# KatherLab/STAMP

Measured on AMD Instinct MI355X. Metric: tiles/sec encoded (224x224, ViT-L/14), higher is better.
Workload: dtype f16

## Files before the change

stamp_amd/csrc/api.hip:

```cpp
#include "gemm_kernel.h"
#include <stdlib.h>
#include <atomic>
#include <mutex>

namespace amds {

static thread_local char g_err[512] = "";

void set_error(const char* fmt, ...) {
    va_list ap;
    va_start(ap, fmt);
    vsnprintf(g_err, sizeof(g_err), fmt, ap);
    va_end(ap);
}

int hip_fail(hipError_t e, const char* what) {
    set_error("HIP error %d (%s) in %s", (int)e, hipGetErrorString(e), what);
    return AMDS_ERR_HIP;
}

}
struct amds_ctx {
    int device = -1;
    int refs = 0;
// ... 294 lines not shown
    set_error("amds_gemm_batched: bad dtype %d", dtype);
    return AMDS_ERR_INVALID;
}

extern "C" int amds_wgrad_tn(const void* dy, long ld_dy, const void* x, long ld_x, long tokens, int N, int K, int split_k, int dtype, float* part,
                             void* stream) {
    AMDS_REQUIRE(dy && x && part, "amds_wgrad_tn: null pointer");
    AMDS_REQUIRE(tokens > 0 && N > 0 && K > 0 && split_k > 0 && split_k <= 65535, "amds_wgrad_tn: bad shape");
    AMDS_REQUIRE(N % 256 == 0 && K % 256 == 0, "amds_wgrad_tn: needs N %% 256 == 0 and K %% 256 == 0 (N=%d K=%d)", N, K);
    AMDS_REQUIRE(ld_dy % 8 == 0 && ld_x % 8 == 0 && ld_dy >= N && ld_x >= K, "amds_wgrad_tn: bad pitches");
    AMDS_REQUIRE(((uintptr_t)dy & 15) == 0 && ((uintptr_t)x & 15) == 0 && ((uintptr_t)part & 15) == 0, "amds_wgrad_tn: pointers must be 16-byte aligned");
    const long unit = 64L * split_k;
    const long chunk = (tokens + unit - 1) / unit * 64;
    AMDS_REQUIRE((chunk + 63) * std::max(ld_dy, ld_x) * 2 < (1L << 31), "amds_wgrad_tn: one split's operand span is beyond the 2 GB a buffer descriptor addresses (raise split_k)");
    EpiArgs ep;
    ep.out = part; ep.ldo = K; ep.bias = nullptr; ep.scale = nullptr; ep.pos = nullptr; ep.np = ep.T = ep.P = 0; ep.acc_scale = 1.0f;
    ep.bsA = chunk * ld_dy; ep.bsW = chunk * ld_x; ep.bsOut = (long)N * K; ep.nbatch = split_k; ep.ktot = tokens;
    hipStream_t st = (hipStream_t)stream;
    ProfScope prof(PROF_GEMM, 2.0 * tokens * (double)N * K, st);
    if (dtype == AMDS_F16) return gemm_dispatch<f16>(15, AMDS_EPI_BIAS_F32, dy, ld_dy, x, ld_x, N, K, (int)chunk, ep, st);
    if (dtype == AMDS_BF16) return gemm_dispatch<bf16>(15, AMDS_EPI_BIAS_F32, dy, ld_dy, x, ld_x, N, K, (int)chunk, ep, st);
    set_error("amds_wgrad_tn: bad dtype %d", dtype);
    return AMDS_ERR_INVALID;
}

extern "C" int amds_gemm_lnfold(const void* A, long lda, const void* W, long ldw, int M, int N, int K, int dtype, int epi, void* out,
                                long ldo, const float* bias, const float* scale, void* xh, float* rowpart, const float* rowstat,
                                const float* colsum, void* stream) {
    AMDS_REQUIRE(A && W && out, "amds_gemm_lnfold: null pointer");
    AMDS_REQUIRE(M >= 0 && N > 0 && K > 0 && K % 64 == 0 && N % 256 == 0, "amds_gemm_lnfold: needs K %% 64 == 0 and N %% 256 == 0 (M=%d N=%d K=%d)", M, N, K);
    AMDS_REQUIRE(lda % 8 == 0 && ldw % 8 == 0 && lda >= K && ldw >= K && ldo % 4 == 0, "amds_gemm_lnfold: bad pitches");
    AMDS_REQUIRE(((uintptr_t)A & 15) == 0 && ((uintptr_t)W & 15) == 0 && ((uintptr_t)out & 15) == 0 && ((uintptr_t)xh & 15) == 0,
                 "amds_gemm_lnfold: pointers must be 16-byte aligned");
    const bool producer = xh || rowpart, consumer = rowstat || colsum;
    AMDS_REQUIRE(producer != consumer, "amds_gemm_lnfold: either (xh, rowpart) [RESIDUAL] or (rowstat, colsum) [BIAS / BIAS_GELU / SWIGLU]");
    if (producer) {
        AMDS_REQUIRE(epi == AMDS_EPI_RESIDUAL && xh && rowpart, "amds_gemm_lnfold: the producer form is the RESIDUAL epilogue with xh AND rowpart");
    } else {
        AMDS_REQUIRE((epi == AMDS_EPI_BIAS || epi == AMDS_EPI_BIAS_GELU || epi == AMDS_EPI_SWIGLU) && rowstat && colsum && bias,
                     "amds_gemm_lnfold: the consumer form is BIAS / BIAS_GELU / SWIGLU with rowstat, colsum AND bias");
    }
    if (M == 0) return AMDS_OK;
    EpiArgs ep;
    ep.out = out; ep.ldo = ldo; ep.bias = bias; ep.scale = scale; ep.pos = nullptr; ep.np = ep.T = ep.P = 0; ep.acc_scale = 1.0f;
    ep.xh = xh; ep.rowpart = rowpart; ep.rowstat = rowstat; ep.colsum = colsum;
    hipStream_t st = (hipStream_t)stream;
    ProfScope prof(PROF_GEMM, 2.0 * M * (double)N * K, st);
    if (dtype == AMDS_F16) return gemm_dispatch<f16>(12, epi, A, lda, W, ldw, M, N, K, ep, st);
    if (dtype == AMDS_BF16) return gemm_dispatch<bf16>(12, epi, A, lda, W, ldw, M, N, K, ep, st);
    set_error("amds_gemm_lnfold: bad dtype %d", dtype);
    return AMDS_ERR_INVALID;
}

extern "C" int amds_gemm_lnfold_planes(const void* A, long lda, const void* W, long ldw, int M, int N, int K, void* hi, void* lo, long ld,
                                       const float* bias, const float* scale, float* rowpart, void* stream) {
    AMDS_REQUIRE(A && W && hi && lo && rowpart, "amds_gemm_lnfold_planes: null pointer");
    AMDS_REQUIRE(M >= 0 && N > 0 && K > 0 && K % 64 == 0 && N % 256 == 0, "amds_gemm_lnfold_planes: needs K %% 64 == 0 and N %% 256 == 0 (M=%d N=%d K=%d)", M, N, K);
    AMDS_REQUIRE(lda % 8 == 0 && ldw % 8 == 0 && lda >= K && ldw >= K && ld % 4 == 0 && ld >= N, "amds_gemm_lnfold_planes: bad pitches");
    AMDS_REQUIRE(((uintptr_t)A & 15) == 0 && ((uintptr_t)W & 15) == 0 && ((uintptr_t)hi & 15) == 0 && ((uintptr_t)lo & 15) == 0,
                 "amds_gemm_lnfold_planes: pointers must be 16-byte aligned");
    AMDS_REQUIRE(hi != lo && A != hi && A != lo, "amds_gemm_lnfold_planes: the planes are updated in place and must not alias each other or A");
    if (M == 0) return AMDS_OK;
    EpiArgs ep;
    ep.out = hi; ep.ldo = ld; ep.bias = bias; ep.scale = scale; ep.pos = nullptr; ep.np = ep.T = ep.P = 0; ep.acc_scale = 1.0f;
    ep.xh = hi; ep.xl = lo; ep.rowpart = rowpart;
    hipStream_t st = (hipStream_t)stream;
    ProfScope prof(PROF_GEMM, 2.0 * M * (double)N * K, st);
    return gemm_dispatch<f16>(12, AMDS_EPI_RESIDUAL, A, lda, W, ldw, M, N, K, ep, st);
}

extern "C" long amds_gemm_persist_launches(void) { return g_gemm_persist_launches.load(std::memory_order_relaxed); }

extern "C" int amds_gemm_ex(int cfg, const void* A, long lda, const void* W, long ldw, int M, int N, int K, int dtype,
                            int epi, void* out, long ldo, const float* bias, const float* scale, const float* pos,
                            int np, int T, int P, float acc_scale, void* stream) {
    return gemm_impl(cfg, A, lda, W, ldw, M, N, K, dtype, epi, out, ldo, bias, scale, pos, np, T, P, acc_scale, stream);
}
```

stamp_amd/csrc/common.h:

```cpp
#pragma once
#include <type_traits>
#include <hip/hip_runtime.h>
#include <stdint.h>
#include <stdio.h>
#include <stdarg.h>
#include <string.h>
#include <atomic>
#include "../../include/amdstamp.h"

namespace amds {

typedef _Float16 f16;
typedef __bf16 bf16;
typedef _Float16 f16x4 __attribute__((ext_vector_type(4)));
typedef _Float16 f16x8 __attribute__((ext_vector_type(8)));
typedef __bf16 bf16x4 __attribute__((ext_vector_type(4)));
typedef __bf16 bf16x8 __attribute__((ext_vector_type(8)));
typedef float f32x4 __attribute__((ext_vector_type(4)));
typedef float f32x16 __attribute__((ext_vector_type(16)));
typedef unsigned int u32x4 __attribute__((ext_vector_type(4)));
typedef unsigned int u32x2 __attribute__((ext_vector_type(2)));
typedef int i32x4 __attribute__((ext_vector_type(4)));

void set_error(const char* fmt, ...);
// ... 124 lines not shown
}
__device__ __forceinline__ f32x2 gelu_erf_poly2(f32x2 x) {
    f32x2 q[1] = {x};
    gelu_erf_poly2_n<1>(q);
    return q[0];
}
__device__ __forceinline__ float silu(float x) { return x * __builtin_amdgcn_rcpf(1.0f + __expf(-x)); }
__device__ __forceinline__ f32x2 silu_mul2(f32x2 g, f32x2 v) {
    const f32x2 a = g * f32x2{-1.44269504088896340736f, -1.44269504088896340736f};
    const f32x2 d = f32x2{__builtin_amdgcn_exp2f(a[0]), __builtin_amdgcn_exp2f(a[1])} + f32x2{1.0f, 1.0f};
    return g * f32x2{__builtin_amdgcn_rcpf(d[0]), __builtin_amdgcn_rcpf(d[1])} * v;
}

__device__ __forceinline__ float half_wave_sum(float v) {
    v += __builtin_bit_cast(float, __builtin_amdgcn_update_dpp(0, __builtin_bit_cast(int, v), 0xB1, 0xF, 0xF, true));
    v += __builtin_bit_cast(float, __builtin_amdgcn_update_dpp(0, __builtin_bit_cast(int, v), 0x4E, 0xF, 0xF, true));
    v += __builtin_bit_cast(float, __builtin_amdgcn_update_dpp(0, __builtin_bit_cast(int, v), 0x141, 0xF, 0xF, true));
    v += __builtin_bit_cast(float, __builtin_amdgcn_update_dpp(0, __builtin_bit_cast(int, v), 0x140, 0xF, 0xF, true));
    v += __builtin_bit_cast(float, __builtin_amdgcn_ds_swizzle(__builtin_bit_cast(int, v), 0x401F));
    return v;
}
__device__ __forceinline__ f32x2 half_wave_sum8(const f32x2 (&v)[8], int lane) {
    auto dpp = [](float x, auto ctrl_c) {
        return __builtin_bit_cast(float, __builtin_amdgcn_update_dpp(0, __builtin_bit_cast(int, x), decltype(ctrl_c)::value, 0xF, 0xF, true));
    };
    typedef std::integral_constant<int, 0x140> MIRROR;
    typedef std::integral_constant<int, 0x141> HALF_MIRROR;
    typedef std::integral_constant<int, 0xB1> XOR1;
    typedef std::integral_constant<int, 0x4E> XOR2;
    const bool b3 = lane & 8, b2 = lane & 4;
    f32x2 a[4], b[2], c;
#pragma unroll
    for (int j = 0; j < 4; ++j)
#pragma unroll
        for (int e = 0; e < 2; ++e) {
            float lo = v[j][e], hi4 = v[4 + j][e];
            asm volatile("s_nop 1\n\tv_permlane16_swap_b32 %0, %1\n\ts_nop 1" : "+v"(lo), "+v"(hi4));
            a[j][e] = lo + hi4;
        }
#pragma unroll
    for (int j = 0; j < 2; ++j) {
        const f32x2 keep = b3 ? a[2 + j] : a[j], send = b3 ? a[j] : a[2 + j];
        b[j] = keep + f32x2{dpp(send[0], MIRROR{}), dpp(send[1], MIRROR{})};
    }
    {
        const f32x2 keep = b2 ? b[1] : b[0], send = b2 ? b[0] : b[1];
        c = keep + f32x2{dpp(send[0], HALF_MIRROR{}), dpp(send[1], HALF_MIRROR{})};
    }
    c += f32x2{dpp(c[0], XOR1{}), dpp(c[1], XOR1{})};
    c += f32x2{dpp(c[0], XOR2{}), dpp(c[1], XOR2{})};
    return c;
}

__device__ __forceinline__ float half_wave_max(float v) {
    v = fmaxf(v, __builtin_bit_cast(float, __builtin_amdgcn_update_dpp(0, __builtin_bit_cast(int, v), 0xB1, 0xF, 0xF, true)));
    v = fmaxf(v, __builtin_bit_cast(float, __builtin_amdgcn_update_dpp(0, __builtin_bit_cast(int, v), 0x4E, 0xF, 0xF, true)));
    v = fmaxf(v, __builtin_bit_cast(float, __builtin_amdgcn_update_dpp(0, __builtin_bit_cast(int, v), 0x141, 0xF, 0xF, true)));
    v = fmaxf(v, __builtin_bit_cast(float, __builtin_amdgcn_update_dpp(0, __builtin_bit_cast(int, v), 0x140, 0xF, 0xF, true)));
    v = fmaxf(v, __builtin_bit_cast(float, __builtin_amdgcn_ds_swizzle(__builtin_bit_cast(int, v), 0x401F)));
    return v;
}

__device__ __forceinline__ float wave_sum(float v) {
#pragma unroll
    for (int o = 32; o > 0; o >>= 1) v += __shfl_xor(v, o, 64);
    return v;
}
__device__ __forceinline__ float wave_max(float v) {
#pragma unroll
    for (int o = 32; o > 0; o >>= 1) v = fmaxf(v, __shfl_xor(v, o, 64));
    return v;
}

__device__ __forceinline__ float dist_sqrt(float x) { return __builtin_amdgcn_sqrtf(x); }
__device__ __host__ __forceinline__ uint32_t fmix32(uint32_t h) {
    h ^= h >> 16; h *= 0x85EBCA6Bu; h ^= h >> 13; h *= 0xC2B2AE35u; h ^= h >> 16;
    return h;
}
__device__ __host__ __forceinline__ uint32_t drop_rowkey(uint64_t seed, uint32_t stream, uint64_t row) {
    const uint32_t a = fmix32((uint32_t)seed ^ (uint32_t)row ^ (stream * 0x9E3779B1u));
    return fmix32(a + (uint32_t)(seed >> 32) + (uint32_t)(row >> 32) * 0x7FEB352Du);
}
__device__ __host__ __forceinline__ uint32_t drop_mix(uint32_t h) {
    h ^= h >> 16; h *= 0xC2B2AE35u; h ^= h >> 16;
    return h;
}
__device__ __host__ __forceinline__ uint32_t drop_pair_bits(uint32_t rowkey, uint32_t pair) { return drop_mix(rowkey ^ (pair * 0x9E3779B1u)); }
__device__ __host__ __forceinline__ bool drop_keep(uint32_t pair_bits, int odd, uint32_t thr16) {
    return ((pair_bits >> (odd ? 16 : 0)) & 0xFFFFu) >= thr16;
}
__device__ __forceinline__ bool drop_keep_flat(uint64_t seed, uint32_t stream, long idx, uint32_t thr16) {
    const uint32_t key = drop_rowkey(seed, stream, (uint64_t)(idx >> 16));
    return drop_keep(drop_pair_bits(key, (uint32_t)(idx & 0xFFFF) >> 1), (int)(idx & 1), thr16);
}
static inline uint32_t drop_thr16(float p) { const long t = lroundf(p * 65536.0f); return (uint32_t)(t < 0 ? 0 : (t > 65535 ? 65535 : t)); }
static inline float drop_scale(uint32_t thr16) { return 65536.0f / (float)(65536u - thr16); }

typedef const __attribute__((address_space(1))) void* gptr_t;
typedef __attribute__((address_space(3))) void* lptr_t;
__device__ __forceinline__ void glds16(const void* g, void* lds_wave_base) {
    __builtin_amdgcn_global_load_lds((gptr_t)g, (lptr_t)lds_wave_base, 16, 0, 0);
}

__device__ __forceinline__ void bufl16(__amdgpu_buffer_rsrc_t rsrc, void* lds_wave_base, int voffset, int soffset) {
    __builtin_amdgcn_raw_ptr_buffer_load_lds(rsrc, (lptr_t)lds_wave_base, 16, voffset, soffset, 0, 0);
}
// ... 56 lines not shown
```

stamp_amd/csrc/gemm_4w16.h:

```cpp
#pragma once
#include <algorithm>
#include <type_traits>
#include "gemm_kernel.h"

namespace amds {

__device__ __forceinline__ f32x4 agpr_read(const f32x4& a) {
    f32x4 v;
    asm("v_accvgpr_read_b32 %0, %1" : "=v"(v[0]) : "a"(a[0]));
    asm("v_accvgpr_read_b32 %0, %1" : "=v"(v[1]) : "a"(a[1]));
    asm("v_accvgpr_read_b32 %0, %1" : "=v"(v[2]) : "a"(a[2]));
    asm("v_accvgpr_read_b32 %0, %1" : "=v"(v[3]) : "a"(a[3]));
    return v;
}

template <int N> struct NextTilePieces : std::integral_constant<int, N> {};
template <typename C> struct is_next_tile : std::false_type {};
template <int N> struct is_next_tile<NextTilePieces<N>> : std::true_type {};

template <typename T, int EPI, int P3 = 6, int P0 = 6, bool SPREAD = true, int PRL = 0, int PRS = 0, bool STREAM = false, bool PERSIST = false, bool TN = false>
__global__ void __launch_bounds__(256) __attribute__((amdgpu_waves_per_eu(1, 1)))
gemm_4w16_kernel(const T* __restrict__ A, long lda, const T* __restrict__ W, long ldw, int M, int N, int K,
                 EpiArgs ep, int tiles_m, int tiles_n) {
    typedef typename Act<T>::vec8 vec8;
    typedef typename Act<T>::vec4 vec4;
    constexpr int BM = 256, BN = 256, BK = 64, NT = 256;
    constexpr int ROWB = BK * 2;
    constexpr int A_BYTES = BM * ROWB, STAGE = (BM + BN) * ROWB;
    constexpr int FI = 8, FJ = 8;
    constexpr int GROUP_M = 8;

    extern __shared__ __attribute__((aligned(16))) char smem[];
#ifdef AMDS_GEMM_TRACE
    unsigned long long tr_t[4] = {0, 0, 0, 0}, tr_rt0 = __builtin_amdgcn_s_memrealtime();
    int tr_round = 0;
#define AMDS_GEMM_STAMP(k)                             \
    do {                                               \
        __builtin_amdgcn_sched_barrier(0);             \
        tr_t[k] = __builtin_amdgcn_s_memtime();        \
        __builtin_amdgcn_sched_barrier(0);             \
    } while (0)
#define AMDS_GEMM_TRACE_WRITE()                                                                                                            \
    do {                                                                                                                                   \
        if (ep.pos != nullptr && threadIdx.x == 0) {                                                                                       \
            unsigned long long* rec = reinterpret_cast<unsigned long long*>(const_cast<float*>(ep.pos)) +                                  \
                                      ((long)blockIdx.x * ((ntiles + (int)gridDim.x - 1) / (int)gridDim.x) + tr_round) * 8;                \
            rec[0] = tr_t[0]; rec[1] = tr_t[1]; rec[2] = tr_t[2]; rec[3] = tr_t[3];                                                        \
            rec[4] = (unsigned long long)__builtin_amdgcn_s_getreg(63492) | ((unsigned long long)__builtin_amdgcn_s_getreg(63508) << 32);  \
            rec[5] = (unsigned long long)ti;                                                                                               \
            rec[6] = tr_rt0; rec[7] = __builtin_amdgcn_s_memrealtime();                                                                    \
        }                                                                                                                                  \
        ++tr_round;                                                                                                                        \
    } while (0)
    AMDS_GEMM_STAMP(0);
#else
#define AMDS_GEMM_STAMP(k) do { } while (0)
#define AMDS_GEMM_TRACE_WRITE() do { } while (0)
#endif

    const int tid = threadIdx.x;
    const int lane = tid & 63;
    const int wave = __builtin_amdgcn_readfirstlane(tid >> 6);
    const int wm = wave >> 1, wn = wave & 1;
    const int l15 = lane & 15, kb = lane >> 4;
    const int l31 = lane & 31, hi = lane >> 5;

    static_assert(!PERSIST || (STREAM && !TN && P3 >= 0 && PRL + PRS == 0 && (EPI == AMDS_EPI_BIAS || EPI == AMDS_EPI_BIAS_GELU || EPI == AMDS_EPI_BIAS_RELU)),
                  "gemm_4w16: the persistent form is the streamed 16-bit epilogue on SCHED 0");
    int tm, tn;
    auto tile_of = [&](int bid, int nwg, int& tm_, int& tn_) {
        const int xcd = bid & 7, q = nwg >> 3, r = nwg & 7;
        const int t = (xcd < r ? xcd * (q + 1) : r * (q + 1) + (xcd - r) * q) + (bid >> 3);
        const int group = GROUP_M * tiles_n;
        const int g = t / group, first_m = g * GROUP_M;
        const int gm = min(tiles_m - first_m, GROUP_M);
        const int rr = t - g * group;
        tm_ = first_m + rr % gm;
        tn_ = rr / gm;
    };
    const int ntiles = PERSIST ? tiles_m * tiles_n : (int)gridDim.x;
    int ti = blockIdx.x;
    tile_of(ti, ntiles, tm, tn);
    int m0 = tm * BM, n0 = tn * BN;
    int par = 0;
    if (ep.nbatch > 1) {
        const long by = blockIdx.y;
        A += by * ep.bsA;
        W += by * ep.bsW;
        constexpr bool F32O = (EPI == AMDS_EPI_RESIDUAL || EPI == AMDS_EPI_BIAS_F32 || EPI == AMDS_EPI_BIAS_GELU_F32 || EPI == AMDS_EPI_BIAS_RELU_F32);
        if (F32O) ep.out = reinterpret_cast<float*>(ep.out) + by * ep.bsOut;
        else ep.out = reinterpret_cast<T*>(ep.out) + by * ep.bsOut;
    }

    int rows_a = min(BM, M - m0);
    const long tn_valid = TN ? (ep.ktot > 0 ? min((long)K, ep.ktot - (long)blockIdx.y * K) : (long)K) : 0;
    __amdgpu_buffer_rsrc_t rsrc_a = TN ? __builtin_amdgcn_make_buffer_rsrc(const_cast<T*>(A + m0), 0, tn_valid > 0 ? (int)(((tn_valid - 1) * lda + BM) * 2) : 0, 0x00020000)
                                             : __builtin_amdgcn_make_buffer_rsrc(const_cast<T*>(A + (long)m0 * lda), 0, (int)((((long)rows_a - 1) * lda + K) * 2), 0x00020000);
    __amdgpu_buffer_rsrc_t rsrc_w = TN ? __builtin_amdgcn_make_buffer_rsrc(const_cast<T*>(W + n0), 0, tn_valid > 0 ? (int)(((tn_valid - 1) * ldw + BN) * 2) : 0, 0x00020000)
                                             : __builtin_amdgcn_make_buffer_rsrc(const_cast<T*>(W + (long)n0 * ldw), 0, (int)(((long)(BN - 1) * ldw + K) * 2), 0x00020000);
    int voff[16];
#pragma unroll
    for (int it = 0; it < 16; ++it) {
        if constexpr (TN) {
            const int c = (it & 7) * NT + tid, row = c >> 5, pos = c & 31, g = (row & 3) | ((row >> 1) & 4);
            voff[it] = (int)(((long)row * (it < 8 ? lda : ldw) + (pos ^ (g << 1)) * 8) * 2);
        } else {
            const int c = (it & 7) * NT + tid, row = c >> 3, cp = c & 7, sc = cp ^ ((row >> 1) & 7);
            voff[it] = (int)(((long)row * (it < 8 ? lda : ldw) + sc * 8) * 2);
        }
    }
    auto issue_to = [&](const __amdgpu_buffer_rsrc_t& ra, const __amdgpu_buffer_rsrc_t& rw, char* st, int koff, int koff_w, int lo, int hi_) {
#pragma unroll
        for (int it = 0; it < 16; ++it)
            if (it >= lo && it < hi_) {
                if (it < 8) {
                    __builtin_amdgcn_raw_ptr_buffer_load_lds(ra, (lptr_t)(st + ((it & 7) * NT + wave * 64) * 16), 16, voff[it], koff, 0, 0);
                } else {
                    __builtin_amdgcn_raw_ptr_buffer_load_lds(rw, (lptr_t)(st + A_BYTES + ((it & 7) * NT + wave * 64) * 16), 16, voff[it], koff_w,
                                                             0, 0);
                }
            }
// ... 292 lines not shown
    for (int i = 0; i < FI; ++i) {
        if (i == 0)
            asm volatile("s_nop 15\n\ts_nop 15" : "+a"(acc[i][0]), "+a"(acc[i][1]), "+a"(acc[i][2]), "+a"(acc[i][3]), "+a"(acc[i][4]),
                         "+a"(acc[i][5]), "+a"(acc[i][6]), "+a"(acc[i][7]));
        else
            asm volatile("" : "+a"(acc[i][0]), "+a"(acc[i][1]), "+a"(acc[i][2]), "+a"(acc[i][3]), "+a"(acc[i][4]), "+a"(acc[i][5]),
                         "+a"(acc[i][6]), "+a"(acc[i][7]));
    }
    __builtin_amdgcn_sched_barrier(0);

    constexpr bool F16OUT = (EPI == AMDS_EPI_BIAS || EPI == AMDS_EPI_BIAS_GELU || EPI == AMDS_EPI_BIAS_RELU);
    static_assert(epi_is_staged<EPI>() || EPI == AMDS_EPI_SWIGLU, "gemm_4w16: staged epilogues and SWIGLU");
    if constexpr (EPI == AMDS_EPI_SWIGLU) {
        const float as = ep.acc_scale;
#pragma unroll
        for (int i = 0; i < FI; ++i) {
            const int row = wm * 128 + i * 16 + l15;
#pragma unroll
            for (int q = 0; q < 2; ++q)
#pragma unroll
                for (int t = 0; t < 2; ++t) {
                    f32x4 gt = agpr_read(acc[i][4 * q + t]), vl = agpr_read(acc[i][4 * q + 2 + t]);
                    if (lnf) {
                        gt = gt * rs[i][0] + (cs[4 * q + t] * rs[i][1] + cb[4 * q + t]);
                        vl = vl * rs[i][0] + (cs[4 * q + 2 + t] * rs[i][1] + cb[4 * q + 2 + t]);
                    } else if (!bias_in_acc) {
                        const f32x4 bg = *reinterpret_cast<const f32x4*>(ep.bias + n0 + wn * 128 + (4 * q + t) * 16 + 4 * kb);
                        const f32x4 bv = *reinterpret_cast<const f32x4*>(ep.bias + n0 + wn * 128 + (4 * q + 2 + t) * 16 + 4 * kb);
                        gt = gt * as + bg;
                        vl = vl * as + bv;
                    }
                    f32x4 o;
                    {
                        const f32x2 o01 = silu_mul2(f32x2{gt[0], gt[1]}, f32x2{vl[0], vl[1]}), o23 = silu_mul2(f32x2{gt[2], gt[3]}, f32x2{vl[2], vl[3]});
                        o = f32x4{o01[0], o01[1], o23[0], o23[1]};
                    }
                    const int hcol = wn * 64 + q * 32 + t * 16 + 4 * kb;
                    const int chunk = hcol >> 3, half = ((hcol >> 2) & 1) * 8;
                    *reinterpret_cast<vec4*>(smem + row * 256 + ((chunk ^ (row & 15)) << 4) + half) = Act<T>::from_f32x4(o);
                }
        }
        __syncthreads();
        const int l15r = lane & 15, rsub = lane >> 4;
#pragma unroll 4
        for (int it = 0; it < 16; ++it) {
            const int row = wave * 64 + it * 4 + rsub;
            const u32x4 v = *reinterpret_cast<const u32x4*>(smem + row * 256 + l15r * 16);
            const int chunk = l15r ^ (row & 15);
            if (m0 + row < M)
                *reinterpret_cast<u32x4*>(reinterpret_cast<T*>(ep.out) + (long)(m0 + row) * ep.ldo + n0 / 2 + chunk * 8) = v;
        }
        return;
    }
    if constexpr (EPI == AMDS_EPI_RESIDUAL) {
        if (rmw_fast) {
            const int rows_o = min(BM, M - m0);
            rsrc_o = __builtin_amdgcn_make_buffer_rsrc(reinterpret_cast<float*>(ep.out) + (long)m0 * ep.ldo + n0, 0,
                                                       (int)((((long)rows_o - 1) * ep.ldo + BN) * 4), 0x00020000);
#pragma unroll
            for (int h = 0; h < 2; ++h)
#pragma unroll
                for (int u = 0; u < 8; ++u)
                    offu[h][u] = (wave * 64 + 2 * u + hi) * ldo4 + (((l31 >> 4) ^ h) << 9) + (((l31 & 15) ^ (2 * u + hi)) << 4);
            const __amdgpu_buffer_rsrc_t rsrc_h = __builtin_amdgcn_make_buffer_rsrc(
                ep.xh ? reinterpret_cast<T*>(ep.xh) + (long)m0 * ep.ldo + n0 : reinterpret_cast<T*>(ep.out), 0,
                ep.xh ? (int)((((long)rows_o - 1) * ep.ldo + BN) * 2) : 0, 0x00020000);
            const __amdgpu_buffer_rsrc_t rsrc_l = __builtin_amdgcn_make_buffer_rsrc(
                ep.xl ? reinterpret_cast<T*>(ep.xl) + (long)m0 * ep.ldo + n0 : reinterpret_cast<T*>(ep.out), 0,
                ep.xl ? (int)((((long)rows_o - 1) * ep.ldo + BN) * 2) : 0, 0x00020000);
            const int np_part = N / 128;
            auto run = [&](auto has_scale_c, auto lnp_c, auto pl_c) {
                constexpr bool HS = decltype(has_scale_c)::value, LNP = decltype(lnp_c)::value, PL = decltype(pl_c)::value;
                auto load_prev = [&](int pass, int b8) {
                    if constexpr (PL) {
                        int rowoff = b8 * 16 * ldo4 + pass * 256;
                        asm volatile("" : "+s"(rowoff));
#pragma unroll
                        for (int u = 0; u < 8; ++u) {
                            const int o = (offu[b8 & 1][u] + rowoff) >> 1;
                            const u32x2 ph = __builtin_bit_cast(u32x2, __builtin_amdgcn_raw_buffer_load_b64(rsrc_h, o, 0, 0));
                            const u32x2 pl = __builtin_bit_cast(u32x2, __builtin_amdgcn_raw_buffer_load_b64(rsrc_l, o, 0, 0));
                            old[b8][u] = __builtin_bit_cast(f32x4, u32x4{ph[0], ph[1], pl[0], pl[1]});
                        }
                    } else {
                        load_old(pass, b8);
                    }
                };
                f32x4 sc[4];
                auto load_scale = [&](int pass) {
                    if constexpr (HS) {
#pragma unroll
                        for (int jj = 0; jj < 4; ++jj)
                            sc[jj] = *reinterpret_cast<const f32x4*>(ep.scale + n0 + wn * 128 + (pass * 4 + jj) * 16 + 4 * kb);
                    }
                };
                load_scale(0);
#pragma unroll
                for (int b8 = 0; b8 < 4; ++b8) load_prev(0, b8);
#pragma unroll
                for (int pass = 0; pass < 2; ++pass) {
#pragma unroll
                    for (int i = 0; i < FI; ++i) {
                        const int row = wm * 128 + i * 16 + l15;
#pragma unroll
                        for (int jj = 0; jj < 4; ++jj) {
                            f32x4 v = agpr_read(acc[i][pass * 4 + jj]);
// ... 29 lines not shown
                                } else {
                                    old4 = __builtin_convertvector(h4, f32x4) + __builtin_convertvector(l4, f32x4);
                                }
                                v[u] += old4;
                            } else {
                                v[u] += old[b8][u];
                                __builtin_amdgcn_raw_buffer_store_b128(__builtin_bit_cast(u32x4, v[u]), rsrc_o, offu[b8 & 1][u] + rowoff, 0, 0);
                            }
                        }
                        if constexpr (LNP) {
                            f32x2 ss[8];
#pragma unroll
                            for (int u = 0; u < 8; ++u) {
                                const vec4 c = Act<T>::from_f32x4(v[u]);
                                __builtin_amdgcn_raw_buffer_store_b64(__builtin_bit_cast(u32x2, c), rsrc_h, (offu[b8 & 1][u] + rowoff) >> 1, 0, 0);
                                if constexpr (PL) {
                                    f32x4 rest;
                                    if constexpr (std::is_same<T, f16>::value) {
                                        const u32x2 cu = __builtin_bit_cast(u32x2, c);
                                        rest = f32x4{mix_sub_fh<0>(v[u][0], cu[0]), mix_sub_fh<1>(v[u][1], cu[0]), mix_sub_fh<0>(v[u][2], cu[1]), mix_sub_fh<1>(v[u][3], cu[1])};
                                    } else {
                                        rest = v[u] - __builtin_convertvector(c, f32x4);
                                    }
                                    const vec4 cl = Act<T>::from_f32x4(rest);
                                    __builtin_amdgcn_raw_buffer_store_b64(__builtin_bit_cast(u32x2, cl), rsrc_l, (offu[b8 & 1][u] + rowoff) >> 1, 0, 0);
                                }
                                ss[u] = f32x2{(v[u][0] + v[u][1]) + (v[u][2] + v[u][3]),
                                              fmaf(v[u][0], v[u][0], v[u][1] * v[u][1]) + fmaf(v[u][2], v[u][2], v[u][3] * v[u][3])};
                            }
                            const f32x2 tot = half_wave_sum8(ss, l31);
                            const int urow = ((l31 >> 4) & 1) * 4 + ((l31 >> 3) & 1) * 2 + ((l31 >> 2) & 1);
                            const int prow = m0 + wave * 64 + b8 * 16 + 2 * urow + hi;
                            if ((l31 & 3) == 0 && prow < M)
                                *reinterpret_cast<f32x2*>(ep.rowpart + ((long)prow * np_part + tn * 2 + pass) * 2) = tot;
                        }
                        if (pass == 0) load_prev(1, b8);
                        __builtin_amdgcn_sched_barrier(0);
                    }
                    if (pass == 0) {
                        asm volatile("s_waitcnt lgkmcnt(0)" ::: "memory");
                        __builtin_amdgcn_sched_barrier(0);
                        __builtin_amdgcn_s_barrier();
                        __builtin_amdgcn_sched_barrier(0);
                    }
                }
            };
            if (ep.xl) {
                if (ep.scale) run(std::true_type{}, std::true_type{}, std::true_type{}); else run(std::false_type{}, std::true_type{}, std::true_type{});
            } else if (ep.xh) {
                if (ep.scale) run(std::true_type{}, std::true_type{}, std::false_type{}); else run(std::false_type{}, std::true_type{}, std::false_type{});
            } else {
                if (ep.scale) run(std::true_type{}, std::false_type{}, std::false_type{}); else run(std::false_type{}, std::false_type{}, std::false_type{});
            }
            return;
        }
    }
    if constexpr (F16OUT && STREAM) {
        EpiArgs epv = ep;
        if (bias_in_acc || lnf) epv.bias = nullptr;
        EpiCols<FJ> cols;
        if constexpr (PERSIST) {
#pragma unroll
            for (int j = 0; j < FJ; ++j) asm volatile("" : "=v"(cols.bias[j]));
        }
        epi_cols_load<EPI>(epv, cols, [&](int j) { return n0 + wn * 128 + j * 16 + 4 * kb; });
        if constexpr (PERSIST) {
            __builtin_amdgcn_sched_barrier(0);
            __builtin_amdgcn_s_waitcnt(0x0F70);
            __builtin_amdgcn_sched_barrier(0);
        }
        const int rows_o = min(BM, M - m0);
        const __amdgpu_buffer_rsrc_t rsrc_s = __builtin_amdgcn_make_buffer_rsrc(reinterpret_cast<T*>(ep.out) + (long)m0 * ep.ldo + n0, 0,
                                                                                (int)((((long)rows_o - 1) * ep.ldo + BN) * 2), 0x00020000);
        char* slab = smem + (PERSIST ? ((nk - 1 + par) & 1) * STAGE : 0) + wave * 8192;
        int wr_base = l15 * 256 + (((kb & 1) ^ (l15 & 1)) << 3);
        int wr_x = (kb >> 1) ^ ((l15 >> 1) & 7);
        int rd_base = kb * 512 + ((l15 ^ kb) << 4);
        int ldo2 = (int)ep.ldo * 2;
        int st_base = (wm * 128 + 2 * kb) * ldo2 + (wn * 128 + l15 * 8) * 2;
        if constexpr (PERSIST) {
            asm volatile("" : "+v"(wr_base), "+v"(wr_x), "+v"(rd_base), "+v"(st_base), "+s"(ldo2));
        }
        auto run = [&](auto mode_c) {
            constexpr int MODE = decltype(mode_c)::value;
            u32x4 rd[4];
            f32x4 b0n[PERSIST && MODE == 1 ? FJ : 1];
            if constexpr (PERSIST && MODE == 1) {
#pragma unroll
                for (int j = 0; j < FJ; ++j) b0n[j] = f32x4{0.f, 0.f, 0.f, 0.f};
                if (bias_in_acc) {
#pragma unroll
                    for (int j = 0; j < FJ; ++j) b0n[j] = *reinterpret_cast<const f32x4*>(ep.bias + n0n + wn * 128 + j * 16 + 4 * kb);
                }
            }
#pragma unroll
            for (int s = 0; s <= FI; ++s) {
                if (s < FI) {
                    char* wp = slab + (s & 1) * 4096 + wr_base;
#pragma unroll
                    for (int j = 0; j < FJ; j += 2) {
                        f32x4 v0 = agpr_read(acc[s][j]), v1 = agpr_read(acc[s][j + 1]);
                        if constexpr (MODE == 2) {
                            if constexpr (LNC) {
                                v0 = v0 * rs[s][0] + (cs[j] * rs[s][1] + cb[j]);
                                v1 = v1 * rs[s][0] + (cs[j + 1] * rs[s][1] + cb[j + 1]);
                                epi_value_pair<EPI, true, true>(epv, cb[j], cb[j], cb[j + 1], cb[j + 1], v0, v1);
// ... 131 lines not shown
                u32x4 v[8];
#pragma unroll
                for (int u = 0; u < 8; ++u) {
                    const int row = wave * 64 + (b8 * 8 + u) * 2 + hi;
                    v[u] = *reinterpret_cast<const u32x4*>(smem + row * 512 + l31 * 16);
                    if ((u >> 2) & 1) v[u] = u32x4{v[u][2], v[u][3], v[u][0], v[u][1]};
                }
#pragma unroll
                for (int u = 0; u < 8; ++u) {
                    const int row = wave * 64 + (b8 * 8 + u) * 2 + hi;
                    const int chunk = l31 ^ (row & 31);
                    if (m0 + row < M)
                        *reinterpret_cast<u32x4*>(reinterpret_cast<T*>(ep.out) + (long)(m0 + row) * ep.ldo + n0 + chunk * 8) = v[u];
                }
            } else {
                f32x4 v[8], o[8];
#pragma unroll
                for (int u = 0; u < 8; ++u) {
                    const int row = wave * 64 + (b8 * 8 + u) * 2 + hi;
                    const int chunk = l31 ^ (row & 31);
                    const int n = n0 + (chunk >> 4) * 128 + pass * 64 + (chunk & 15) * 4;
                    v[u] = *reinterpret_cast<const f32x4*>(smem + row * 512 + l31 * 16);
                    if constexpr (EPI == AMDS_EPI_RESIDUAL)
                        o[u] = *reinterpret_cast<const f32x4*>(reinterpret_cast<const float*>(ep.out) +
                                                               (long)min(m0 + row, M - 1) * ep.ldo + n);
                }
#pragma unroll
                for (int u = 0; u < 8; ++u) {
                    const int row = wave * 64 + (b8 * 8 + u) * 2 + hi;
                    const int chunk = l31 ^ (row & 31);
                    const int n = n0 + (chunk >> 4) * 128 + pass * 64 + (chunk & 15) * 4;
                    if constexpr (EPI == AMDS_EPI_RESIDUAL) v[u] += o[u];
                    if (m0 + row < M)
                        *reinterpret_cast<f32x4*>(reinterpret_cast<float*>(ep.out) + (long)(m0 + row) * ep.ldo + n) = v[u];
                }
            }
        }
    }
}

static inline int gemm_persist_grid(int tiles) {
    int g = device_cu_count() & ~7;
    const char* e = getenv("AMDS_GEMM_PERSIST_WGS");
    if (e && *e) g = std::min(g, atoi(e) & ~7);
    return std::min(tiles, std::max(g, 8));
}

template <typename T, int EPI, bool SPREAD = true, int P3 = 6, int P0 = 6, int PRL = 0, int PRS = 0, bool STREAM = false, bool PERSIST = false, bool TN = false>
static int launch_gemm_4w16(const void* A, long lda, const void* W, long ldw, int M, int N, int K, const EpiArgs& ep,
                            hipStream_t st) {
    if constexpr (!epi_is_staged<EPI>() && EPI != AMDS_EPI_SWIGLU) {
        return launch_gemm_4w64<T, EPI>(A, lda, W, ldw, M, N, K, ep, st);
    } else {
        constexpr int LDS = 2 * (256 + 256) * 128;
        constexpr bool STR = STREAM && (EPI == AMDS_EPI_BIAS || EPI == AMDS_EPI_BIAS_GELU || EPI == AMDS_EPI_BIAS_RELU);
        if constexpr (STR) {
            if (ep.ldo * 512 >= (1L << 31)) return launch_gemm_4w16<T, EPI, SPREAD, P3, P0, PRL, PRS, false, false, TN>(A, lda, W, ldw, M, N, K, ep, st);
        }
        constexpr bool PER = PERSIST && STR && !TN && P3 >= 0 && PRL + PRS == 0;
        if constexpr (PER) {
            if (ep.nbatch != 1) return launch_gemm_4w16<T, EPI, SPREAD, P3, P0, PRL, PRS, STREAM, false, TN>(A, lda, W, ldw, M, N, K, ep, st);
        }
        constexpr auto kern = gemm_4w16_kernel<T, EPI, P3, P0, SPREAD, PRL, PRS, STR, PER, TN>;
        EpiArgs epp = ep;
        if constexpr (PRL + PRS > 0) {
            static char* scratch = nullptr;
            static size_t scratch_bytes = 0;
            const size_t need = (size_t)cdiv(M, 256) * (N / 256) * (K / 64) * 4096 * (PRL > PRS ? PRL : PRS);
            if (need > scratch_bytes) {
                if (scratch) AMDS_HIP(hipFree(scratch));
                AMDS_HIP(hipMalloc(reinterpret_cast<void**>(&scratch), need));
                scratch_bytes = need;
            }
            epp.pos = reinterpret_cast<const float*>(scratch);
        }
        AMDS_HIP(lds_opt_in<kern>(LDS));
        const int tiles_m = cdiv(M, 256), tiles_n = N / 256;
        int grid = tiles_m * tiles_n;
        if constexpr (PER) {
            grid = gemm_persist_grid(grid);
            g_gemm_persist_launches.fetch_add(1, std::memory_order_relaxed);
        }
        hipLaunchKernelGGL(kern, dim3(grid, ep.nbatch), dim3(256), LDS, st, reinterpret_cast<const T*>(A), lda,
                           reinterpret_cast<const T*>(W), ldw, M, N, K, epp, tiles_m, tiles_n);
        AMDS_LAUNCH_CHECK("gemm_4w16_kernel");
        return AMDS_OK;
    }
}

}
```

stamp_amd/csrc/gemm_kernel.h:

```cpp
#pragma once
#include <stdlib.h>
#include <atomic>
#include <type_traits>
#include "launch.h"

namespace amds {

struct EpiArgs {
    void* out;
    long ldo;
    const float* bias;
    const float* scale;
    const float* pos;
    int np, T, P;
    float acc_scale;
    long bsA = 0, bsW = 0, bsOut = 0;
    int nbatch = 1;
    void* xh = nullptr;
    void* xl = nullptr;
    float* rowpart = nullptr;
    const float* rowstat = nullptr;
    const float* colsum = nullptr;
    long ktot = 0;
};
// ... 298 lines not shown
                        for (int e = 0; e < 4; ++e) {
                            gte[e] = acc[i][j][4 * g + e] * ep.acc_scale + bg[e];
                            val[e] = acc[i][j + 1][4 * g + e] * ep.acc_scale + bv[e];
                            o[e] = Act<T>::from_f32(silu(gte[e]) * val[e]);
                        }
                        *reinterpret_cast<vec4*>(reinterpret_cast<T*>(ep.out) + (long)m * ep.ldo + hcol) = o;
                    }
                }
            } else {
#pragma unroll
                for (int j = 0; j < FN; ++j)
#pragma unroll
                    for (int g = 0; g < 4; ++g) {
                        const int n = n0 + wn * WTN + j * 32 + 8 * g + 4 * hi;
                        epilogue4<EPI, T>(ep, m, n, acc[i][j][4 * g + 0], acc[i][j][4 * g + 1],
                                          acc[i][j][4 * g + 2], acc[i][j][4 * g + 3]);
                    }
            }
        }
    }
    }
}

template <typename T, int BM, int BN, int WM, int WN, int EPI>
static int launch_gemm_cfg(const void* A, long lda, const void* W, long ldw, int M, int N, int K,
                           const EpiArgs& ep, hipStream_t st) {
    constexpr int STAGE = (BM + BN) * 64 * 2;
    constexpr int EPI_LDS = BM * ((BN * 4 / 16) | 1) * 16;
    constexpr int LDS = 2 * STAGE > EPI_LDS ? 2 * STAGE : EPI_LDS;
    constexpr auto kern = gemm_tn_kernel<T, BM, BN, WM, WN, EPI>;
    AMDS_HIP(lds_opt_in<kern>(LDS));
    const int tiles_m = cdiv(M, BM), tiles_n = N / BN;
    hipLaunchKernelGGL(kern, dim3(tiles_m * tiles_n), dim3(64 * WM * WN), LDS, st,
                       reinterpret_cast<const T*>(A), lda, reinterpret_cast<const T*>(W), ldw, M, N, K, ep,
                       tiles_m, tiles_n);
    AMDS_LAUNCH_CHECK("gemm_tn_kernel");
    return AMDS_OK;
}

template <typename T, int EPI>
static int launch_gemm_8p64(const void* A, long lda, const void* W, long ldw, int M, int N, int K, const EpiArgs& ep,
                            hipStream_t st);
template <typename T, int EPI>
static int launch_gemm_4w64(const void* A, long lda, const void* W, long ldw, int M, int N, int K, const EpiArgs& ep,
                            hipStream_t st);
template <typename T, int EPI, bool SPREAD, int P3, int P0, int PRL, int PRS, bool STREAM, bool PERSIST, bool TN>
static int launch_gemm_4w16(const void* A, long lda, const void* W, long ldw, int M, int N, int K, const EpiArgs& ep,
                            hipStream_t st);

static inline bool gemm_epi_stream() {
    const char* e = getenv("AMDS_GEMM_EPI_STREAM");
    return !(e && *e && atoi(e) == 0);
}
inline std::atomic<long> g_gemm_persist_launches{0};
static inline bool gemm_persist() {
    const char* e = getenv("AMDS_GEMM_PERSIST");
    return !(e && *e && atoi(e) == 0);
}

template <typename T, int EPI>
static int launch_gemm(int cfg, const void* A, long lda, const void* W, long ldw, int M, int N, int K,
                       const EpiArgs& ep, hipStream_t st) {
    if (cfg == 10 && N % 256 == 0 && ep.nbatch == 1) return launch_gemm_4w64<T, EPI>(A, lda, W, ldw, M, N, K, ep, st);
    if (cfg == 10) cfg = 8;
    if ((cfg == 12 || cfg == 13 || cfg == 14 || cfg == 16) && N % 256 == 0) {
        const bool stream = cfg != 14 && gemm_epi_stream();
        if (cfg == 13) {
            if (stream) return launch_gemm_4w16<T, EPI, true, -2, 0, 0, 0, true, false, false>(A, lda, W, ldw, M, N, K, ep, st);
            return launch_gemm_4w16<T, EPI, true, -2, 0, 0, 0, false, false, false>(A, lda, W, ldw, M, N, K, ep, st);
        }
        if constexpr (EPI == AMDS_EPI_BIAS || EPI == AMDS_EPI_BIAS_GELU || EPI == AMDS_EPI_BIAS_RELU) {
            if (stream && (cfg == 16 || gemm_persist())) return launch_gemm_4w16<T, EPI, true, 6, 6, 0, 0, true, true, false>(A, lda, W, ldw, M, N, K, ep, st);
        }
        if (stream) return launch_gemm_4w16<T, EPI, true, 6, 6, 0, 0, true, false, false>(A, lda, W, ldw, M, N, K, ep, st);
        return launch_gemm_4w16<T, EPI, true, 6, 6, 0, 0, false, false, false>(A, lda, W, ldw, M, N, K, ep, st);
    }
#ifdef AMDS_GEMM_PROBE
    if constexpr (EPI == AMDS_EPI_BIAS || EPI == AMDS_EPI_BIAS_GELU || EPI == AMDS_EPI_RESIDUAL) {
        if (cfg == 21 && N % 256 == 0) return launch_gemm_4w16<T, EPI, true, 6, 6, 0, 2, false, false, false>(A, lda, W, ldw, M, N, K, ep, st);
        if (cfg == 22 && N % 256 == 0) return launch_gemm_4w16<T, EPI, true, 6, 6, 1, 1, false, false, false>(A, lda, W, ldw, M, N, K, ep, st);
        if (cfg == 23 && N % 256 == 0) return launch_gemm_4w16<T, EPI, true, 6, 6, 4, 4, false, false, false>(A, lda, W, ldw, M, N, K, ep, st);
    }
#endif
    if constexpr (EPI == AMDS_EPI_BIAS_F32) {
        if (cfg == 15 && N % 256 == 0 && M % 256 == 0) return launch_gemm_4w16<T, EPI, true, 6, 6, 0, 0, false, false, true>(A, lda, W, ldw, M, N, K, ep, st);
    }
    if (cfg == 15) { set_error("amds_gemm: kernel 15 (token-major operands) takes the BIAS_F32 epilogue and M, N multiples of 256"); return AMDS_ERR_INVALID; }
    if (cfg == 12 || cfg == 13 || cfg == 14 || cfg == 16) cfg = 8;

    if (cfg == 8 && N % 256 == 0) return launch_gemm_8p64<T, EPI>(A, lda, W, ldw, M, N, K, ep, st);
    if (cfg == 8) cfg = 0;
    if (cfg == 0 && N % 128 != 0) cfg = 1;
    switch (cfg) {
        case 0: return launch_gemm_cfg<T, 128, 128, 2, 2, EPI>(A, lda, W, ldw, M, N, K, ep, st);
        case 1:
            if constexpr (EPI == AMDS_EPI_SWIGLU || EPI == AMDS_EPI_PATCH) {
                set_error("amds_gemm: the 128x96 tile has no SWIGLU / PATCH epilogue");
                return AMDS_ERR_INVALID;
            } else {
                if (N % 96 != 0) { set_error("amds_gemm: kernel 1 needs N %% 96 == 0 (N=%d)", N); return AMDS_ERR_INVALID; }
                return launch_gemm_cfg<T, 128, 96, 4, 1, EPI>(A, lda, W, ldw, M, N, K, ep, st);
            }
    }
    set_error("amds_gemm: unknown tile config %d", cfg);
    return AMDS_ERR_INVALID;
}

template <typename T>
int gemm_dispatch(int cfg, int epi, const void* A, long lda, const void* W, long ldw, int M, int N, int K,
                  const EpiArgs& ep, hipStream_t st);

#define AMDS_GEMM_DISPATCH_IMPL(T)                                                                        \
    template <>                                                                                           \
    int gemm_dispatch<T>(int cfg, int epi, const void* A, long lda, const void* W, long ldw, int M, int N, \
                         int K, const EpiArgs& ep, hipStream_t st) {                                      \
        switch (epi) {                                                                                    \
            case AMDS_EPI_BIAS: return launch_gemm<T, AMDS_EPI_BIAS>(cfg, A, lda, W, ldw, M, N, K, ep, st); \
            case AMDS_EPI_BIAS_GELU: return launch_gemm<T, AMDS_EPI_BIAS_GELU>(cfg, A, lda, W, ldw, M, N, K, ep, st); \
            case AMDS_EPI_BIAS_RELU: return launch_gemm<T, AMDS_EPI_BIAS_RELU>(cfg, A, lda, W, ldw, M, N, K, ep, st); \
            case AMDS_EPI_RESIDUAL: return launch_gemm<T, AMDS_EPI_RESIDUAL>(cfg, A, lda, W, ldw, M, N, K, ep, st); \
            case AMDS_EPI_BIAS_F32: return launch_gemm<T, AMDS_EPI_BIAS_F32>(cfg, A, lda, W, ldw, M, N, K, ep, st); \
            case AMDS_EPI_SWIGLU: return launch_gemm<T, AMDS_EPI_SWIGLU>(cfg, A, lda, W, ldw, M, N, K, ep, st); \
            case AMDS_EPI_PATCH: return launch_gemm<T, AMDS_EPI_PATCH>(cfg, A, lda, W, ldw, M, N, K, ep, st); \
            case AMDS_EPI_BIAS_GELU_F32: return launch_gemm<T, AMDS_EPI_BIAS_GELU_F32>(cfg, A, lda, W, ldw, M, N, K, ep, st); \
            case AMDS_EPI_BIAS_RELU_F32: return launch_gemm<T, AMDS_EPI_BIAS_RELU_F32>(cfg, A, lda, W, ldw, M, N, K, ep, st); \
// ... 7 lines not shown
```

Before: 6214.

## Add streamed and persistent residual-planes epilogue to the 4w16 GEMM

Adds a streamed epilogue for the fp16 hi/lo residual-planes producer GEMM. It stages accumulators through a per-wave LDS slab, prefetches the old planes with buffer loads a few row-groups ahead, and writes new hi/lo planes together with per-row sum and sum-of-squares partials, reduced with DPP. It also lets the persistent tile loop drive this epilogue, so the next tile's loads overlap the current store phase. Both paths are on by default through env flags. The cost is extra LDS, more register pressure and added code complexity.

```diff
diff --git a/stamp_amd/csrc/api.hip b/stamp_amd/csrc/api.hip
--- a/stamp_amd/csrc/api.hip
+++ b/stamp_amd/csrc/api.hip
@@ -370,6 +370,11 @@
     return AMDS_ERR_INVALID;
 }
 
+#ifdef AMDS_GEMM_TRACE
+static const float* g_gemm_trace_buffer = nullptr;
+extern "C" void amds_gemm_trace_buffer(void* p) { g_gemm_trace_buffer = reinterpret_cast<const float*>(p); }
+#endif
+
 extern "C" int amds_gemm_lnfold_planes(const void* A, long lda, const void* W, long ldw, int M, int N, int K, void* hi, void* lo, long ld,
                                        const float* bias, const float* scale, float* rowpart, void* stream) {
     AMDS_REQUIRE(A && W && hi && lo && rowpart, "amds_gemm_lnfold_planes: null pointer");
@@ -382,6 +387,9 @@
     EpiArgs ep;
     ep.out = hi; ep.ldo = ld; ep.bias = bias; ep.scale = scale; ep.pos = nullptr; ep.np = ep.T = ep.P = 0; ep.acc_scale = 1.0f;
     ep.xh = hi; ep.xl = lo; ep.rowpart = rowpart;
+#ifdef AMDS_GEMM_TRACE
+    ep.pos = g_gemm_trace_buffer;
+#endif
     hipStream_t st = (hipStream_t)stream;
     ProfScope prof(PROF_GEMM, 2.0 * M * (double)N * K, st);
     return gemm_dispatch<f16>(12, AMDS_EPI_RESIDUAL, A, lda, W, ldw, M, N, K, ep, st);
diff --git a/stamp_amd/csrc/common.h b/stamp_amd/csrc/common.h
--- a/stamp_amd/csrc/common.h
+++ b/stamp_amd/csrc/common.h
@@ -200,6 +200,34 @@
     return c;
 }
 
+__device__ __forceinline__ f32x2 row16_sum8(const f32x2 (&v)[8], int lane) {
+    auto dpp = [](float x, auto ctrl_c) {
+        return __builtin_bit_cast(float, __builtin_amdgcn_update_dpp(0, __builtin_bit_cast(int, x), decltype(ctrl_c)::value, 0xF, 0xF, true));
+    };
+    typedef std::integral_constant<int, 0x140> MIRROR;
+    typedef std::integral_constant<int, 0x141> HALF_MIRROR;
+    typedef std::integral_constant<int, 0xB1> XOR1;
+    typedef std::integral_constant<int, 0x4E> XOR2;
+    const bool b3 = lane & 8, b2 = lane & 4, b0 = lane & 1;
+    f32x2 a[4], b[2], c;
+#pragma unroll
+    for (int j = 0; j < 4; ++j) {
+        const f32x2 keep = b3 ? v[4 + j] : v[j], send = b3 ? v[j] : v[4 + j];
+        a[j] = keep + f32x2{dpp(send[0], MIRROR{}), dpp(send[1], MIRROR{})};
+    }
+#pragma unroll
+    for (int j = 0; j < 2; ++j) {
+        const f32x2 keep = b2 ? a[2 + j] : a[j], send = b2 ? a[j] : a[2 + j];
+        b[j] = keep + f32x2{dpp(send[0], HALF_MIRROR{}), dpp(send[1], HALF_MIRROR{})};
+    }
+    {
+        const f32x2 keep = b0 ? b[1] : b[0], send = b0 ? b[0] : b[1];
+        c = keep + f32x2{dpp(send[0], XOR1{}), dpp(send[1], XOR1{})};
+    }
+    c += f32x2{dpp(c[0], XOR2{}), dpp(c[1], XOR2{})};
+    return c;
+}
+
 __device__ __forceinline__ float half_wave_max(float v) {
     v = fmaxf(v, __builtin_bit_cast(float, __builtin_amdgcn_update_dpp(0, __builtin_bit_cast(int, v), 0xB1, 0xF, 0xF, true)));
     v = fmaxf(v, __builtin_bit_cast(float, __builtin_amdgcn_update_dpp(0, __builtin_bit_cast(int, v), 0x4E, 0xF, 0xF, true)));
diff --git a/stamp_amd/csrc/gemm_4w16.h b/stamp_amd/csrc/gemm_4w16.h
--- a/stamp_amd/csrc/gemm_4w16.h
+++ b/stamp_amd/csrc/gemm_4w16.h
@@ -65,8 +65,9 @@
     const int l15 = lane & 15, kb = lane >> 4;
     const int l31 = lane & 31, hi = lane >> 5;
 
-    static_assert(!PERSIST || (STREAM && !TN && P3 >= 0 && PRL + PRS == 0 && (EPI == AMDS_EPI_BIAS || EPI == AMDS_EPI_BIAS_GELU || EPI == AMDS_EPI_BIAS_RELU)),
-                  "gemm_4w16: the persistent form is the streamed 16-bit epilogue on SCHED 0");
+    static_assert(!PERSIST || (STREAM && !TN && P3 >= 0 && PRL + PRS == 0 &&
+                               (EPI == AMDS_EPI_BIAS || EPI == AMDS_EPI_BIAS_GELU || EPI == AMDS_EPI_BIAS_RELU || EPI == AMDS_EPI_RESIDUAL)),
+                  "gemm_4w16: the persistent form is a streamed epilogue on SCHED 0");
     int tm, tn;
     auto tile_of = [&](int bid, int nwg, int& tm_, int& tn_) {
         const int xcd = bid & 7, q = nwg >> 3, r = nwg & 7;
@@ -465,6 +466,161 @@
         }
         return;
     }
+    if constexpr (EPI == AMDS_EPI_RESIDUAL && STREAM) {
+        static_assert(std::is_same<T, f16>::value && !TN && PRL + PRS == 0, "gemm_4w16: the streamed residual epilogue is the fp16 planes producer");
+        __builtin_amdgcn_sched_barrier(0);
+        __builtin_amdgcn_s_waitcnt(0x0F70);
+        __builtin_amdgcn_sched_barrier(0);
+        const int rows_o = min(BM, M - m0);
+        int ldo2 = (int)ep.ldo * 2;
+        if constexpr (PERSIST) asm volatile("" : "+s"(ldo2));
+        const __amdgpu_buffer_rsrc_t rsrc_h = __builtin_amdgcn_make_buffer_rsrc(reinterpret_cast<T*>(ep.xh) + (long)m0 * ep.ldo + n0, 0,
+                                                                                (int)((((long)rows_o - 1) * ep.ldo + BN) * 2), 0x00020000);
+        const __amdgpu_buffer_rsrc_t rsrc_l = __builtin_amdgcn_make_buffer_rsrc(reinterpret_cast<T*>(ep.xl) + (long)m0 * ep.ldo + n0, 0,
+                                                                                (int)((((long)rows_o - 1) * ep.ldo + BN) * 2), 0x00020000);
+        char* slab = smem + (PERSIST ? ((nk - 1 + par) & 1) * STAGE : 0) + wave * 16384;
+        float* part = reinterpret_cast<float*>(smem + 2 * STAGE);
+        int wr_base = l15 * 512;
+        int rd_base = hi * 512 + l31 * 16;
+        if constexpr (PERSIST) asm volatile("" : "+v"(wr_base), "+v"(rd_base));
+        int offp[8];
+#pragma unroll
+        for (int u = 0; u < 8; ++u) offp[u] = (wm * 128 + 2 * u + hi) * ldo2 + wn * 256 + ((l31 ^ (2 * u + hi)) << 3);
+        const int np_part = N / 128;
+        auto run = [&](auto has_scale_c) {
+            constexpr bool HS = decltype(has_scale_c)::value;
+            f32x4 sc[HS ? FJ : 1];
+            if constexpr (HS) {
+#pragma unroll
+                for (int j = 0; j < FJ; ++j) sc[j] = *reinterpret_cast<const f32x4*>(ep.scale + n0 + wn * 128 + j * 16 + 4 * kb);
+            }
+            f32x4 b0n[PERSIST ? FJ : 1];
+            u32x4 prev[3][8];
+            auto load_prev = [&](int s) {
+                int rowoff = s * 16 * ldo2;
+                asm volatile("" : "+s"(rowoff));
+#pragma unroll
+                for (int u = 0; u < 8; ++u) {
+                    const u32x2 ph = __builtin_bit_cast(u32x2, __builtin_amdgcn_raw_buffer_load_b64(rsrc_h, offp[u] + rowoff, 0, 0));
+                    const u32x2 pl = __builtin_bit_cast(u32x2, __builtin_amdgcn_raw_buffer_load_b64(rsrc_l, offp[u] + rowoff, 0, 0));
+                    prev[s % 3][u] = u32x4{ph[0], ph[1], pl[0], pl[1]};
+                }
+            };
+            load_prev(0);
+            load_prev(1);
+            f32x4 v[8];
+#pragma unroll
+            for (int s = 0; s <= FI; ++s) {
+                if (s < FI) {
+                    char* wp = slab + (s & 1) * 8192 + wr_base;
+#pragma unroll
+                    for (int j = 0; j < FJ; ++j) {
+                        f32x4 a = agpr_read(acc[s][j]);
+                        if constexpr (HS) a *= sc[j];
+                        *reinterpret_cast<f32x4*>(wp + (((j * 4 + kb) ^ l15) << 4)) = a;
+                    }
+                    if (s >= 1 && s + 1 < FI) load_prev(s + 1);
+                    if constexpr (PERSIST) {
+                        if (s == FI - 1) {
+#pragma unroll
+                            for (int j = 0; j < FJ; ++j) b0n[j] = f32x4{0.f, 0.f, 0.f, 0.f};
+                            if (bias_in_acc) {
+#pragma unroll
+                                for (int j = 0; j < FJ; ++j) b0n[j] = *reinterpret_cast<const f32x4*>(ep.bias + n0n + wn * 128 + j * 16 + 4 * kb);
+                            }
+                        }
+                    }
+                }
+                __builtin_amdgcn_sched_barrier(0);
+                if (s > 0) {
+                    const int t = s - 1;
+                    int rowoff = t * 16 * ldo2;
+                    asm volatile("" : "+s"(rowoff));
+                    f32x2 ss[8];
+#pragma unroll
+                    for (int u = 0; u < 8; ++u) {
+                        const u32x4 o = prev[t % 3][u];
+                        const f32x4 old4 = f32x4{mix_add_hh<0, 0>(o[0], o[2]), mix_add_hh<1, 1>(o[0], o[2]), mix_add_hh<0, 0>(o[1], o[3]), mix_add_hh<1, 1>(o[1], o[3])};
+                        v[u] += old4;
+                        const vec4 c = Act<T>::from_f32x4(v[u]);
+                        __builtin_amdgcn_raw_buffer_store_b64(__builtin_bit_cast(u32x2, c), rsrc_h, offp[u] + rowoff, 0, 0);
+                        const u32x2 cu = __builtin_bit_cast(u32x2, c);
+                        const f32x4 rest = f32x4{mix_sub_fh<0>(v[u][0], cu[0]), mix_sub_fh<1>(v[u][1], cu[0]), mix_sub_fh<0>(v[u][2], cu[1]), mix_sub_fh<1>(v[u][3], cu[1])};
+                        const vec4 cl = Act<T>::from_f32x4(rest);
+                        __builtin_amdgcn_raw_buffer_store_b64(__builtin_bit_cast(u32x2, cl), rsrc_l, offp[u] + rowoff, 0, 0);
+                        ss[u] = f32x2{(v[u][0] + v[u][1]) + (v[u][2] + v[u][3]),
+                                      fmaf(v[u][0], v[u][0], v[u][1] * v[u][1]) + fmaf(v[u][2], v[u][2], v[u][3] * v[u][3])};
+                    }
+                    const f32x2 tot = row16_sum8(ss, lane);
+                    const int urow = ((lane >> 3) & 1) * 4 + ((lane >> 2) & 1) * 2 + (lane & 1);
+                    const int prow = wm * 128 + t * 16 + 2 * urow + hi;
+                    if ((lane & 2) == 0) *reinterpret_cast<f32x2*>(part + ((prow * 2 + ((lane >> 4) & 1)) * 2 + wn) * 2) = tot;
+                }
+                if (s < FI) {
+                    __builtin_amdgcn_fence(__ATOMIC_ACQ_REL, "wavefront");
+                    __builtin_amdgcn_wave_barrier();
+                    const char* rp = slab + (s & 1) * 8192 + rd_base;
+#pragma unroll
+                    for (int u = 0; u < 8; ++u) v[u] = *reinterpret_cast<const f32x4*>(rp + u * 1024);
+                    __builtin_amdgcn_wave_barrier();
+                }
+                __builtin_amdgcn_sched_barrier(0);
+            }
+            if constexpr (PERSIST) {
+#pragma unroll
+                for (int i = 0; i < FI; ++i)
+#pragma unroll
+                    for (int j = 0; j < FJ; ++j) acc[i][j] = b0n[PERSIST ? j : 0];
+            }
+        };
+        if (ep.scale) run(std::true_type{}); else run(std::false_type{});
+        if constexpr (PERSIST) {
+#pragma unroll
+            for (int i = 0; i < FI; ++i) {
+                if (i == FI - 1)
+                    asm volatile("s_nop 7" : "+a"(acc[i][0]), "+a"(acc[i][1]), "+a"(acc[i][2]), "+a"(acc[i][3]), "+a"(acc[i][4]), "+a"(acc[i][5]),
+                                 "+a"(acc[i][6]), "+a"(acc[i][7]));
+                else
+                    asm volatile("" : "+a"(acc[i][0]), "+a"(acc[i][1]), "+a"(acc[i][2]), "+a"(acc[i][3]), "+a"(acc[i][4]), "+a"(acc[i][5]),
+                                 "+a"(acc[i][6]), "+a"(acc[i][7]));
+            }
+        }
+        asm volatile("s_waitcnt lgkmcnt(0)" ::: "memory");
+        __builtin_amdgcn_sched_barrier(0);
+        __builtin_amdgcn_s_barrier();
+        __builtin_amdgcn_sched_barrier(0);
+#pragma unroll
+        for (int e = 0; e < 2; ++e) {
+            const int idx = e * NT + tid, row = idx >> 1;
+            const f32x4 p4 = *reinterpret_cast<const f32x4*>(part + idx * 4);
+            if (m0 + row < M)
+                *reinterpret_cast<f32x2*>(ep.rowpart + ((long)(m0 + row) * np_part + tn * 2 + (idx & 1)) * 2) = f32x2{p4[0] + p4[2], p4[1] + p4[3]};
+        }
+        if constexpr (PERSIST) {
+            AMDS_GEMM_STAMP(3);
+            AMDS_GEMM_TRACE_WRITE();
+            if (!has_next) return;
+            ti += (int)gridDim.x;
+            tn = n0n / BN;
+            m0 = m0n;
+            n0 = n0n;
+            rsrc_a = rsrc_an;
+            rsrc_w = rsrc_wn;
+            par = (par + nk) & 1;
+            AMDS_GEMM_STAMP(0);
+            AMDS_GEMM_STAMP(1);
+            load_frags(0, 0, 0, 0, 16);
+            if (nk > 1) issue_pieces(1, 0, Q3);
+            __builtin_amdgcn_sched_barrier(0);
+            goto next_tile;
+        }
+#ifdef AMDS_GEMM_TRACE
+        asm volatile("s_waitcnt vmcnt(0)" ::: "memory");
+#endif
+        AMDS_GEMM_STAMP(3);
+        AMDS_GEMM_TRACE_WRITE();
+        return;
+    }
     if constexpr (EPI == AMDS_EPI_RESIDUAL) {
         if (rmw_fast) {
             const int rows_o = min(BM, M - m0);
@@ -600,6 +756,11 @@
             } else {
                 if (ep.scale) run(std::true_type{}, std::false_type{}, std::false_type{}); else run(std::false_type{}, std::false_type{}, std::false_type{});
             }
+#ifdef AMDS_GEMM_TRACE
+            asm volatile("s_waitcnt vmcnt(0)" ::: "memory");
+#endif
+            AMDS_GEMM_STAMP(3);
+            AMDS_GEMM_TRACE_WRITE();
             return;
         }
     }
@@ -837,16 +998,21 @@
     if constexpr (!epi_is_staged<EPI>() && EPI != AMDS_EPI_SWIGLU) {
         return launch_gemm_4w64<T, EPI>(A, lda, W, ldw, M, N, K, ep, st);
     } else {
-        constexpr int LDS = 2 * (256 + 256) * 128;
         constexpr bool STR = STREAM && (EPI == AMDS_EPI_BIAS || EPI == AMDS_EPI_BIAS_GELU || EPI == AMDS_EPI_BIAS_RELU);
+        constexpr bool RSTR = STREAM && EPI == AMDS_EPI_RESIDUAL && std::is_same<T, f16>::value && !TN && P3 >= 0 && PRL + PRS == 0;
+        constexpr int LDS = 2 * (256 + 256) * 128 + (RSTR ? 8192 : 0);
+        if constexpr (RSTR) {
+            if (!(ep.xh && ep.xl && ep.rowpart && ep.acc_scale == 1.0f && ep.rowstat == nullptr && ep.nbatch == 1 && ep.ldo * 512 < (1L << 31)))
+                return launch_gemm_4w16<T, EPI, SPREAD, P3, P0, PRL, PRS, false, false, TN>(A, lda, W, ldw, M, N, K, ep, st);
+        }
         if constexpr (STR) {
             if (ep.ldo * 512 >= (1L << 31)) return launch_gemm_4w16<T, EPI, SPREAD, P3, P0, PRL, PRS, false, false, TN>(A, lda, W, ldw, M, N, K, ep, st);
         }
-        constexpr bool PER = PERSIST && STR && !TN && P3 >= 0 && PRL + PRS == 0;
+        constexpr bool PER = PERSIST && (STR || RSTR) && !TN && P3 >= 0 && PRL + PRS == 0;
         if constexpr (PER) {
             if (ep.nbatch != 1) return launch_gemm_4w16<T, EPI, SPREAD, P3, P0, PRL, PRS, STREAM, false, TN>(A, lda, W, ldw, M, N, K, ep, st);
         }
-        constexpr auto kern = gemm_4w16_kernel<T, EPI, P3, P0, SPREAD, PRL, PRS, STR, PER, TN>;
+        constexpr auto kern = gemm_4w16_kernel<T, EPI, P3, P0, SPREAD, PRL, PRS, STR || RSTR, PER, TN>;
         EpiArgs epp = ep;
         if constexpr (PRL + PRS > 0) {
             static char* scratch = nullptr;
diff --git a/stamp_amd/csrc/gemm_kernel.h b/stamp_amd/csrc/gemm_kernel.h
--- a/stamp_amd/csrc/gemm_kernel.h
+++ b/stamp_amd/csrc/gemm_kernel.h
@@ -374,6 +374,14 @@
     const char* e = getenv("AMDS_GEMM_EPI_STREAM");
     return !(e && *e && atoi(e) == 0);
 }
+static inline bool gemm_resid_stream() {
+    const char* e = getenv("AMDS_GEMM_RESID_STREAM");
+    return !(e && *e && atoi(e) == 0);
+}
+static inline bool gemm_resid_persist() {
+    const char* e = getenv("AMDS_GEMM_RESID_PERSIST");
+    return !(e && *e && atoi(e) == 0);
+}
 inline std::atomic<long> g_gemm_persist_launches{0};
 static inline bool gemm_persist() {
     const char* e = getenv("AMDS_GEMM_PERSIST");
@@ -386,13 +394,13 @@
     if (cfg == 10 && N % 256 == 0 && ep.nbatch == 1) return launch_gemm_4w64<T, EPI>(A, lda, W, ldw, M, N, K, ep, st);
     if (cfg == 10) cfg = 8;
     if ((cfg == 12 || cfg == 13 || cfg == 14 || cfg == 16) && N % 256 == 0) {
-        const bool stream = cfg != 14 && gemm_epi_stream();
+        const bool stream = cfg != 14 && (EPI == AMDS_EPI_RESIDUAL ? gemm_resid_stream() : gemm_epi_stream());
         if (cfg == 13) {
             if (stream) return launch_gemm_4w16<T, EPI, true, -2, 0, 0, 0, true, false, false>(A, lda, W, ldw, M, N, K, ep, st);
             return launch_gemm_4w16<T, EPI, true, -2, 0, 0, 0, false, false, false>(A, lda, W, ldw, M, N, K, ep, st);
         }
-        if constexpr (EPI == AMDS_EPI_BIAS || EPI == AMDS_EPI_BIAS_GELU || EPI == AMDS_EPI_BIAS_RELU) {
-            if (stream && (cfg == 16 || gemm_persist())) return launch_gemm_4w16<T, EPI, true, 6, 6, 0, 0, true, true, false>(A, lda, W, ldw, M, N, K, ep, st);
+        if constexpr (EPI == AMDS_EPI_BIAS || EPI == AMDS_EPI_BIAS_GELU || EPI == AMDS_EPI_BIAS_RELU || EPI == AMDS_EPI_RESIDUAL) {
+            if (stream && (cfg == 16 || (gemm_persist() && (EPI != AMDS_EPI_RESIDUAL || gemm_resid_persist())))) return launch_gemm_4w16<T, EPI, true, 6, 6, 0, 0, true, true, false>(A, lda, W, ldw, M, N, K, ep, st);
         }
         if (stream) return launch_gemm_4w16<T, EPI, true, 6, 6, 0, 0, true, false, false>(A, lda, W, ldw, M, N, K, ep, st);
         return launch_gemm_4w16<T, EPI, true, 6, 6, 0, 0, false, false, false>(A, lda, W, ldw, M, N, K, ep, st);
```

Result: faster. 6287, median of 6 (+1.2%).
